# virtualsecureplatform/cuFHE

Measured on AMD Instinct MI355X. Metric: nand_gate_bootstraps_per_sec, higher is better.
Workload: dtype f64

## Files before the change

### cufhe_amd/csrc/kernels.hip.h

```cpp
#pragma once
#include "kernels_common.hip.h"

namespace cufhe_amd {

__global__ __launch_bounds__(kNttThreads) void bk_to_ntt_kernel(
    double* __restrict__ bk_ntt, const uint32_t* __restrict__ bk, size_t polys,
    const NttTables* __restrict__ gt, double n_inverse)
{
    extern __shared__ __attribute__((aligned(16))) char smem[];
    double* tabs = (double*)smem;
    load_tables_to_lds(tabs, gt);
    __syncthreads();
    const int wave = threadIdx.x >> 6, lane = threadIdx.x & 63;
    const size_t poly = (size_t)blockIdx.x * kNttWavesPerBlock + wave;
    if (poly >= polys) return;
    const WaveCtx ctx = make_wave_ctx(smem, kLdsTableBytes + wave * kTileBytes, 0, gt, lane);
    double x[kRegs];
#pragma unroll
    for (int r = 0; r < kRegs; r++) x[r] = (double)(int32_t)bk[poly * kN + lane + 64 * r];
    ntt_forward<false>(x, ctx);
    double2* dst = (double2*)(bk_ntt + poly * kN);
#pragma unroll
    for (int q = 0; q < 8; q++) {
        double2 v;
        v.x = fpf::reduce(fpf::mulmod_wide(x[2 * q], n_inverse));
        v.y = fpf::reduce(fpf::mulmod_wide(x[2 * q + 1], n_inverse));
        dst[q * 64 + lane] = v;
    }
}

__global__ __launch_bounds__(512) void clock_probe_kernel(double* __restrict__ hz_out, double* __restrict__ sink, int iters)
{
    double x = 1.0 + threadIdx.x * 1e-9, y = 0.5;
    const unsigned long long c0 = __builtin_amdgcn_s_memtime(), r0 = __builtin_amdgcn_s_memrealtime();
#pragma unroll 1
    for (int i = 0; i < iters; i++) {
#pragma unroll
        for (int k = 0; k < 16; k++) { x = __builtin_fma(x, 0.999999, y); y = __builtin_fma(y, 0.999999, x); }
    }
    const unsigned long long c1 = __builtin_amdgcn_s_memtime(), r1 = __builtin_amdgcn_s_memrealtime();
    if (x + y == 12345.678) sink[0] = x;
    if ((threadIdx.x & 63) == 0)
        hz_out[blockIdx.x * (blockDim.x >> 6) + (threadIdx.x >> 6)] = (double)(c1 - c0) / (double)(r1 - r0) * 1.0e8;
}

__device__ __forceinline__ void rotate_sub(uint32_t (&temp)[kRegs], const uint32_t (&acc)[kRegs],
                                           char* tile, int lane, uint32_t abar)
{
    const int alo = (int)(abar & (kN - 1));
    const bool ahi = (abar >> kNbit) != 0;
    char* wpos = tile + opaque(4 * lane + (ahi ? 0 : 4 * kN));
    char* wneg = tile + opaque(4 * lane + (ahi ? 4 * kN : 0));
    asm volatile("" ::: "memory");
#pragma unroll
    for (int r = 0; r < kRegs; r++) {
        *(uint32_t*)(wpos + 256 * r) = acc[r];
        *(uint32_t*)(wneg + 256 * r) = 0u - acc[r];
    }
    asm volatile("" ::: "memory");
    const char* rbase = tile + opaque(4 * (lane - alo + kN));
    uint32_t rot[kRegs];
#pragma unroll
    for (int r = 0; r < kRegs; r++) rot[r] = *(const uint32_t*)(rbase + 256 * r);
#pragma unroll
    for (int r = 0; r < kRegs; r++) temp[r] = (rot[r] - acc[r] + decomp_offset()) ^ decomp_signmask();
}

template <class SPEC, int R, bool LAST, bool FIRST = false>
__device__ __forceinline__ void product_into(double& acc, double x, double w)
{
    constexpr bool wide = r4::needs_wide(SPEC::in().v[R]);
    static_assert(!(LAST && FIRST), "a sum of one product has no first row apart from its last");
    if constexpr (LAST) acc = wide ? fpf::mulmod_add_wide(x, w, acc) : fpf::mulmod_add(x, w, acc);
    else if constexpr (FIRST) acc = wide ? fpf::mulmod_wide(x, w) : fpf::mulmod(x, w);
    else acc += wide ? fpf::mulmod_wide(x, w) : fpf::mulmod(x, w);
}
template <class SPEC, bool LAST, bool FIRST, int Q>
__device__ __forceinline__ void pointwise_piece(double (&A0)[kRegs], double (&A1)[kRegs], const double (&x)[kRegs], const double2& b)
{
    if constexpr (Q < 8) {
        product_into<SPEC, 2 * Q, LAST, FIRST>(A0[2 * Q], x[2 * Q], b.x);
        product_into<SPEC, 2 * Q + 1, LAST, FIRST>(A0[2 * Q + 1], x[2 * Q + 1], b.y);
    } else {
        product_into<SPEC, 2 * (Q - 8), LAST, FIRST>(A1[2 * (Q - 8)], x[2 * (Q - 8)], b.x);
        product_into<SPEC, 2 * (Q - 8) + 1, LAST, FIRST>(A1[2 * (Q - 8) + 1], x[2 * (Q - 8) + 1], b.y);
    }
}
template <class SPEC, bool LAST, bool FIRST, int Q = 0>
__device__ __forceinline__ void pointwise_pieces(double (&A0)[kRegs], double (&A1)[kRegs], const double (&x)[kRegs],
                                                 double2 (&b)[16], const char* row_lane)
{
#ifndef CUFHE_AMD_BK_DEPTH
#define CUFHE_AMD_BK_DEPTH 3
#endif
    constexpr int D = CUFHE_AMD_BK_DEPTH;
    if constexpr (Q < 16) {
        if constexpr (Q + D < 16) b[Q + D] = *(const double2*)(row_lane + (Q + D) * 1024);
        __builtin_amdgcn_sched_barrier(0x0006);
        pointwise_piece<SPEC, LAST, FIRST, Q>(A0, A1, x, b[Q]);
        __builtin_amdgcn_sched_barrier(0x0006);
        pointwise_pieces<SPEC, LAST, FIRST, Q + 1>(A0, A1, x, b, row_lane);
    }
}
template <class SPEC, bool LAST, bool FIRST = false>
__device__ __forceinline__ void pointwise_accumulate(double (&A0)[kRegs], double (&A1)[kRegs],
                                                     const double (&x)[kRegs], const char* row_lane)
{
#if defined(CUFHE_AMD_DIAGNOSTIC_BUILD) && defined(CUFHE_AMD_ABL_NO_BK)
    if constexpr (FIRST) {
#pragma unroll
        for (int r = 0; r < kRegs; r++) { A0[r] = 0.0; A1[r] = 0.0; }
    }
#pragma unroll
    for (int q = 0; q < 8; q++) {
        A0[2 * q] += fpf::mulmod_wide(x[2 * q], 1234567.0 + q);
        A0[2 * q + 1] += fpf::mulmod_wide(x[2 * q + 1], 7654321.0 + q);
        A1[2 * q] += fpf::mulmod_wide(x[2 * q], 2234567.0 + q);
        A1[2 * q + 1] += fpf::mulmod_wide(x[2 * q + 1], 8654321.0 + q);
    }
    (void)row_lane;
    return;
#endif
    constexpr int D = CUFHE_AMD_BK_DEPTH;
    double2 b[16];
#pragma unroll
    for (int q = 0; q < D; q++) b[q] = *(const double2*)(row_lane + q * 1024);
    pointwise_pieces<SPEC, LAST, FIRST>(A0, A1, x, b, row_lane);
}

#if defined(CUFHE_AMD_DIAGNOSTIC_BUILD) && defined(CUFHE_AMD_ABL_PHASES)
#define CUFHE_AMD_DIAG_ARG , unsigned long long& diag_wait
#define CUFHE_AMD_DIAG_PASS , diag_wait
#define CUFHE_AMD_ROW_SYNC(R) { const unsigned long long t0_ = __builtin_readcyclecounter(); pipe.sync(R); diag_wait += __builtin_readcyclecounter() - t0_; }
#else
#define CUFHE_AMD_DIAG_ARG
#define CUFHE_AMD_DIAG_PASS
#define CUFHE_AMD_ROW_SYNC(R) pipe.sync(R);
#endif
struct RowPipe {
    const char* src;
    char* buf;
    uint32_t voff;
    int wave, lane, total_rows;
    bool late;
    int row_off;
    __device__ __forceinline__ RowPipe(const char* bk, char* buf_, int wave_, int lane_, int total_rows_, bool late_)
        : src(bk + 2 * wave_ * 1024), buf(buf_), voff(lane_ * 16), wave(wave_), lane(lane_), total_rows(total_rows_), late(late_),
          row_off((kBkRowBuffers - 1) * kBkRowBytes) {}
    static __device__ __forceinline__ int next_off(int off) { return off == (kBkRowBuffers - 1) * kBkRowBytes ? 0 : off + kBkRowBytes; }
    __device__ __forceinline__ void issue(int R)
    {
        if (R < total_rows) {
            char* dst = buf + next_off(row_off) + 2 * wave * 1024;
#pragma unroll
            for (int c = 0; c < 2; c++) lds_dma16(src + c * 1024, voff, dst + c * 1024);
        }
        src += kBkRowBytes;
    }
    __device__ __forceinline__ void sync(int R)
    {
#if defined(CUFHE_AMD_DIAGNOSTIC_BUILD) && defined(CUFHE_AMD_ABL_NO_SYNC)
        (void)R;
        return;
#endif
        lds_dma_wait_all();
        __syncthreads();
        row_off = next_off(row_off);
        issue(R + 1);
    }
    __device__ __forceinline__ const char* row() const { return buf + opaque(row_off + lane * 16); }
};

using BrSpectrum = r4::FwdDigits<(1 << (kBgbit - 1))>::Spectrum;
using BrSums = r4::PointwiseSum<BrSpectrum, kBkRows, true>;
using BrInverse = r4::Inverse<BrSums>;
static_assert(r4::valid(BrSpectrum::in()) && r4::valid(BrSums::in()) && r4::valid(BrInverse::Out::in()),
              "blind_rotate_kernel: the lazy-reduction schedule of the CMux step exceeds the FP64 mantissa");

template <bool FIRST, bool LAST>
__device__ __forceinline__ void cmux_row(double (&A0)[kRegs], double (&A1)[kRegs], const uint32_t (&temp)[kRegs], int d,
                                         const WaveCtx& ctx, RowPipe& pipe, int row, const TuFwdPinned& tuf CUFHE_AMD_DIAG_ARG)
{
    constexpr int kDigitMax = 1 << (kBgbit - 1);
    const uint32_t pos = 32 - (d + 1) * kBgbit;
    double x[kRegs];
#pragma unroll
    for (int r = 0; r < kRegs; r++)
        x[r] = (double)(int32_t)__builtin_amdgcn_sbfe(temp[r], pos, (uint32_t)kBgbit);
    double twb[kTbCount];
    ntt_forward_digits_a_r4<kDigitMax, true>(x, ctx, &tuf, &twb);
    if (pipe.late) CUFHE_AMD_ROW_SYNC(row)
    ntt_forward_digits_bc_r4<kDigitMax, false, true>(x, ctx, twb);
    if (!pipe.late) CUFHE_AMD_ROW_SYNC(row)
    pointwise_accumulate<BrSpectrum, LAST, FIRST>(A0, A1, x, pipe.row());
}

template <bool FIRST_COMPONENT, bool LAST_COMPONENT>
__device__ __forceinline__ void cmux_component(double (&A0)[kRegs], double (&A1)[kRegs],
                                               const uint32_t (&accj)[kRegs], const WaveCtx& ctx,
                                               char* tile, int lane, uint32_t abar,
                                               RowPipe& pipe, int first_row, const TuFwdPinned& tuf CUFHE_AMD_DIAG_ARG)
{
    uint32_t temp[kRegs];
    rotate_sub(temp, accj, tile, lane, abar);
    static_assert(kL >= 2, "the first and the last row of a component are two rows");
    constexpr int lo = FIRST_COMPONENT ? 1 : 0, hi = LAST_COMPONENT ? kL - 1 : kL;
    if constexpr (FIRST_COMPONENT) cmux_row<true, false>(A0, A1, temp, 0, ctx, pipe, first_row, tuf CUFHE_AMD_DIAG_PASS);
#pragma unroll 1
    for (int d = lo; d < hi; d++) cmux_row<false, false>(A0, A1, temp, d, ctx, pipe, first_row + d, tuf CUFHE_AMD_DIAG_PASS);
    if constexpr (LAST_COMPONENT) cmux_row<false, true>(A0, A1, temp, kL - 1, ctx, pipe, first_row + kL - 1, tuf CUFHE_AMD_DIAG_PASS);
}

template <bool TWB_LOADED>
__device__ __forceinline__ void inverse_and_add(double (&A)[kRegs], uint32_t (&accj)[kRegs], const WaveCtx& ctx,
                                                const double (&twc)[kTcCount], double (&twb)[kTbCount])
{
    ntt_inverse_r4_tw<BrSums, false, TWB_LOADED>(A, ctx, twc, twb);
    lift_add<BrInverse::Out>(accj, A);
}

template <bool TABLE>
__global__ __launch_bounds__(kBrThreads, 2) void blind_rotate_kernel(
    const LinDesc* __restrict__ descs, int count, const double* __restrict__ bk_ntt,
    const NttTables* __restrict__ gt, int steps, uint32_t* __restrict__ acc_dump, int active, const uint32_t* __restrict__ tvs,
    const uint32_t* const* __restrict__ tables)
{
    extern __shared__ __attribute__((aligned(16))) char smem[];
    double* tabs = (double*)(smem + kBrLdsTables);
    load_packed_tables_to_lds(tabs, gt);
    const int wave = __builtin_amdgcn_readfirstlane(threadIdx.x >> 6);
    const int lane = threadIdx.x & 63;
    const int g = blockIdx.x * active + wave;
    char* tile = smem + kBrLdsTiles + wave * kTileBytes;
    uint16_t* abar_lds = (uint16_t*)(smem + kBrLdsAbar + wave * kAbarBytes);
    const WaveCtx ctx = make_wave_ctx_packed(smem, kBrLdsTiles + wave * kTileBytes, kBrLdsTables, gt, lane);
    RowPipe pipe((const char*)bk_ntt, smem + kBrLdsBk, wave, lane, steps * kBkRows, wave >= kBrWavesPerBlock / 2);
    pipe.issue(0);
    if (wave >= active || g >= count) {
        __syncthreads();
#pragma unroll 1
        for (int R = 0; R < pipe.total_rows; R++) pipe.sync(R);
        return;
    }

    const LinDesc d = descs[g];
    uint32_t bword = 0;
#pragma unroll
    for (int rr = 0; rr < 10; rr++) {
        const int i = lane + 64 * rr;
        uint32_t c = 0;
        if (i <= kLvl0N) c = (uint32_t)d.ca * d.in0[i] + (uint32_t)d.cb * d.in1[i];
        if (rr == 9) bword = c;
        if (i < kLvl0N) abar_lds[i] = (uint16_t)((c + (1u << (32 - 2 - kNbit))) >> (32 - 1 - kNbit));
    }
    bword = __builtin_amdgcn_readlane(bword, kLvl0N - 64 * 9) + d.off;
    const uint32_t bbar = 2 * kN - (bword >> (32 - 1 - kNbit));

    uint32_t acc0[kRegs], acc1[kRegs];
#pragma unroll
    for (int r = 0; r < kRegs; r++) {
        const uint32_t e = lane + 64 * r;
        acc0[r] = 0;
        const bool neg = (bbar != 2 * kN) && ((e < (bbar & (kN - 1))) != ((bbar >> kNbit) != 0));
        acc1[r] = neg ? 0u - kMu : kMu;
    }
    const uint32_t* tab = nullptr;
    if constexpr (TABLE) tab = tables[g];
    if (TABLE && tab) {
        const int s = desc_shift(d.pad);
        uint32_t bb = bbar;
        if (s) {
            for (int i = lane; i < kLvl0N; i += 64) abar_lds[i] = (uint16_t)ms_abar((uint32_t)d.ca * d.in0[i] + (uint32_t)d.cb * d.in1[i], s);
            bb = ms_bbar(bword, s);
        }
#pragma unroll
        for (int r = 0; r < kRegs; r++) {
            acc0[r] = rotated_tv_coef(tab, bb, lane + 64 * r);
            acc1[r] = rotated_tv_coef(tab + kN, bb, lane + 64 * r);
        }
    } else if (d.pad) {
        const uint32_t* tv = desc_tv(tvs, d.pad);
        const int s = desc_shift(d.pad);
        uint32_t bb = bbar;
        if (s) {
            for (int i = lane; i < kLvl0N; i += 64) abar_lds[i] = (uint16_t)ms_abar((uint32_t)d.ca * d.in0[i] + (uint32_t)d.cb * d.in1[i], s);
            bb = ms_bbar(bword, s);
        }
#pragma unroll
        for (int r = 0; r < kRegs; r++) acc1[r] = rotated_tv_coef(tv, bb, lane + 64 * r);
    }
    __syncthreads();
    TuFwdPinned tuf;
    tuf.load(gt);
#if defined(CUFHE_AMD_DIAGNOSTIC_BUILD) && defined(CUFHE_AMD_ABL_PHASES)
    unsigned long long diag_wait = 0;
    const unsigned long long diag_t0 = __builtin_readcyclecounter();
#endif

#pragma unroll 1
    for (int i = 0; i < steps; i++) {
        const uint32_t abar = __builtin_amdgcn_readfirstlane((uint32_t)abar_lds[i]);
        double A0[kRegs], A1[kRegs], inv_twc[kTcCount], inv_twb[kTbCount];
        cmux_component<true, false>(A0, A1, acc0, ctx, tile, lane, abar, pipe, i * kBkRows, tuf CUFHE_AMD_DIAG_PASS);
        cmux_component<false, true>(A0, A1, acc1, ctx, tile, lane, abar, pipe, i * kBkRows + kL, tuf CUFHE_AMD_DIAG_PASS);
        load_packed(inv_twc, ctx.tc_inv);
        inverse_and_add<false>(A0, acc0, ctx, inv_twc, inv_twb);
        inverse_and_add<true>(A1, acc1, ctx, inv_twc, inv_twb);
    }

    if (acc_dump) {
        uint32_t* o = acc_dump + (size_t)g * 2 * kN;
#pragma unroll
        for (int r = 0; r < kRegs; r++) {
            o[lane + 64 * r] = acc0[r];
            o[kN + lane + 64 * r] = acc1[r];
        }
#if defined(CUFHE_AMD_DIAGNOSTIC_BUILD) && defined(CUFHE_AMD_ABL_PHASES)
        if (lane == 0) {
            ((unsigned long long*)o)[0] = __builtin_readcyclecounter() - diag_t0;
            ((unsigned long long*)o)[1] = diag_wait;
        }
#endif
    }
    if (d.out) {
        uint32_t* o = d.out;
#pragma unroll
        for (int r = 0; r < kRegs; r++) {
            const int e = lane + 64 * r;
            if (e == 0) { o[0] = acc0[r]; o[kN] = acc1[r]; }
            else o[kN - e] = 0u - acc0[r];
        }
        if (const int s = desc_shift(d.pad)) {
#pragma unroll
            for (int r = 0; r < kRegs; r++) extract_more(o, 1 << s, lane + 64 * r, acc0[r], acc1[r]);
        }
    }
}

constexpr int kKsWaves = 16;
constexpr int kKsThreads = 64 * kKsWaves;
constexpr int kKsRowPad = 640;
constexpr int kKsPieces = 3;
constexpr int kKsStepBytes = kKsT * kKsNumBase * kKsRowPad * 4;
constexpr int kKsBuffers = 3;
constexpr int kKsDigitSteps = 1024;
constexpr int kKsLdsDigits = kKsWaves * kKsDigitSteps * 2;

struct KsShapeDefault {
    using Desc = LinDesc;
    static constexpr int kn = kN, t = kKsT, row_pad = kKsRowPad, n_out = kLvl0N;
    static constexpr uint32_t koff()
    {
        uint32_t o = 1u << (32 - (1 + kKsBasebit * kKsT));
        for (int i = 1; i <= kKsT; i++) o += ((1u << kKsBasebit) / 2) << (32 - i * kKsBasebit);
        return o;
    }
    static __device__ __forceinline__ uint32_t digit_word(const Desc& d, int j)
    {
        return ((uint32_t)d.ca * d.in0[j] + (uint32_t)d.cb * d.in1[j] + koff()) >> 16;
    }
    static __device__ __forceinline__ uint32_t bprime(const Desc& d) { return (uint32_t)d.ca * d.in0[kn] + (uint32_t)d.cb * d.in1[kn] + d.off; }
};
template <class S>
struct KsDims {
    static constexpr int pairs = (S::row_pad - 512) / 128;
    static constexpr int words = 8 + 2 * pairs;
    static constexpr int step_bytes = S::t * kKsNumBase * S::row_pad * 4;
    static constexpr int dma_pieces = step_bytes / 1024;
    static constexpr int dma_more = dma_pieces - 2 * kKsWaves;
    static constexpr int lds_bytes = kKsLdsDigits + kKsBuffers * step_bytes;
    static constexpr int min_slices = (S::kn + kKsDigitSteps - 1) / kKsDigitSteps;
    static_assert(S::row_pad == 512 || S::row_pad == 640, "a lane owns two quads and at most one pair of a row");
    static_assert(step_bytes % 1024 == 0 && dma_more >= 0 && dma_more <= kKsWaves, "two or three DMA pieces per wave and step");
    static_assert(S::t * kKsBasebit <= 16 && S::n_out < S::row_pad, "digit word of 16 bits; the output fits a row");
    static_assert(lds_bytes <= 160 * 1024, "digit words + three step buffers fit the CU's LDS");
};
static_assert(KsDims<KsShapeDefault>::step_bytes == kKsStepBytes && KsDims<KsShapeDefault>::lds_bytes == 155648, "BASELINE shape");

typedef uint32_t ks_u32x4 __attribute__((ext_vector_type(4)));
typedef uint32_t ks_u32x2 __attribute__((ext_vector_type(2)));
struct KsRow { ks_u32x4 a, b; ks_u32x2 c; };
template <int ROW1, int ROW2, int PAIRS>
__device__ __forceinline__ void ks_digit_load(const uint32_t f, const uint32_t a0, const uint32_t a1, const uint32_t a2, KsRow& r)
{
    if constexpr (PAIRS) {
        asm volatile(
            "s_cmp_eq_u32 %3, 2\n\t"
            "s_cbranch_scc1 .Lks_ld_end_%=\n\t"
            "s_cmp_eq_u32 %3, 0\n\t"
            "s_cbranch_scc1 .Lks_ld_two_%=\n\t"
            "ds_read_b128 %0, %4 offset:%7\n\t"
            "ds_read_b128 %1, %5 offset:%7\n\t"
            "ds_read_b64 %2, %6 offset:%7\n\t"
            "s_branch .Lks_ld_end_%=\n"
            ".Lks_ld_two_%=:\n\t"
            "ds_read_b128 %0, %4 offset:%8\n\t"
            "ds_read_b128 %1, %5 offset:%8\n\t"
            "ds_read_b64 %2, %6 offset:%8\n"
            ".Lks_ld_end_%=:"
            : "=&v"(r.a), "=&v"(r.b), "=&v"(r.c)
            : "s"(f), "v"(a0), "v"(a1), "v"(a2), "n"(ROW1), "n"(ROW2)
            : "memory", "scc");
    } else {
        asm volatile(
            "s_cmp_eq_u32 %2, 2\n\t"
            "s_cbranch_scc1 .Lks_ld_end_%=\n\t"
            "s_cmp_eq_u32 %2, 0\n\t"
            "s_cbranch_scc1 .Lks_ld_two_%=\n\t"
            "ds_read_b128 %0, %3 offset:%5\n\t"
            "ds_read_b128 %1, %4 offset:%5\n\t"
            "s_branch .Lks_ld_end_%=\n"
            ".Lks_ld_two_%=:\n\t"
            "ds_read_b128 %0, %3 offset:%6\n\t"
            "ds_read_b128 %1, %4 offset:%6\n"
            ".Lks_ld_end_%=:"
            : "=&v"(r.a), "=&v"(r.b)
            : "s"(f), "v"(a0), "v"(a1), "n"(ROW1), "n"(ROW2)
            : "memory", "scc");
    }
}
template <int PAIRS>
__device__ __forceinline__ void ks_digit_acc(const uint32_t f, const KsRow& r, uint32_t (&res)[8 + 2 * PAIRS])
{
    if constexpr (PAIRS) {
#define CUFHE_AMD_KS_ALL(OP)                                                                                               \
    OP " %0, %0, %11\n\t" OP " %1, %1, %12\n\t" OP " %2, %2, %13\n\t" OP " %3, %3, %14\n\t" OP " %4, %4, %15\n\t"             \
    OP " %5, %5, %16\n\t" OP " %6, %6, %17\n\t" OP " %7, %7, %18\n\t" OP " %8, %8, %19\n\t" OP " %9, %9, %20\n"
        asm volatile(
            "s_cmp_eq_u32 %10, 2\n\t"
            "s_cbranch_scc1 .Lks_acc_end_%=\n\t"
            "s_cmp_eq_u32 %10, 3\n\t"
            "s_cbranch_scc1 .Lks_acc_sub_%=\n\t"
            CUFHE_AMD_KS_ALL("v_add_u32_e32")
            "\ts_branch .Lks_acc_end_%=\n"
            ".Lks_acc_sub_%=:\n\t"
            CUFHE_AMD_KS_ALL("v_sub_u32_e32")
            ".Lks_acc_end_%=:"
            : "+v"(res[0]), "+v"(res[1]), "+v"(res[2]), "+v"(res[3]), "+v"(res[4]), "+v"(res[5]), "+v"(res[6]), "+v"(res[7]), "+v"(res[8]), "+v"(res[9])
            : "s"(f), "v"(r.a.x), "v"(r.a.y), "v"(r.a.z), "v"(r.a.w), "v"(r.b.x), "v"(r.b.y), "v"(r.b.z), "v"(r.b.w), "v"(r.c.x), "v"(r.c.y)
            : "scc");
#undef CUFHE_AMD_KS_ALL
    } else {
#define CUFHE_AMD_KS_ALL(OP)                                                                                               \
    OP " %0, %0, %9\n\t" OP " %1, %1, %10\n\t" OP " %2, %2, %11\n\t" OP " %3, %3, %12\n\t" OP " %4, %4, %13\n\t"              \
    OP " %5, %5, %14\n\t" OP " %6, %6, %15\n\t" OP " %7, %7, %16\n"
        asm volatile(
            "s_cmp_eq_u32 %8, 2\n\t"
            "s_cbranch_scc1 .Lks_acc_end_%=\n\t"
            "s_cmp_eq_u32 %8, 3\n\t"
            "s_cbranch_scc1 .Lks_acc_sub_%=\n\t"
            CUFHE_AMD_KS_ALL("v_add_u32_e32")
            "\ts_branch .Lks_acc_end_%=\n"
            ".Lks_acc_sub_%=:\n\t"
            CUFHE_AMD_KS_ALL("v_sub_u32_e32")
            ".Lks_acc_end_%=:"
            : "+v"(res[0]), "+v"(res[1]), "+v"(res[2]), "+v"(res[3]), "+v"(res[4]), "+v"(res[5]), "+v"(res[6]), "+v"(res[7])
            : "s"(f), "v"(r.a.x), "v"(r.a.y), "v"(r.a.z), "v"(r.a.w), "v"(r.b.x), "v"(r.b.y), "v"(r.b.z), "v"(r.b.w)
            : "scc");
#undef CUFHE_AMD_KS_ALL
    }
}
template <int I, int N, class F>
__device__ __forceinline__ void ks_for(F&& f)
{
    if constexpr (I < N) {
        f(std::integral_constant<int, I>{});
        ks_for<I + 1, N>(f);
    }
}
__device__ __forceinline__ uint32_t ks_field(const uint32_t dj, const int k) { return (dj >> (16 - (k + 1) * kKsBasebit)) & ((1u << kKsBasebit) - 1); }
template <class S>
__device__ __forceinline__ void ks_load_all(const uint32_t dj, const uint32_t (&pb)[3], KsRow (&r)[S::t])
{
// ... 401 lines not shown
```

### cufhe_amd/csrc/ntt_wave.h

```cpp
#pragma once
#include <hip/hip_runtime.h>
#include "fpfield.h"
#include "ntt_r4.h"
#include "ntt_tables.h"

namespace cufhe_amd {

constexpr int kRegs = 16;
constexpr int kTileSlots = 66 * 16;
constexpr int kTileBytes = kTileSlots * 8;

constexpr double forward_digit_spectrum_bound(double digit_max)
{
    const double s1 = digit_max * (1.0 + fpf::ROOT4 + fpf::ROOT8 + fpf::ROOT8 * fpf::ROOT8 * fpf::ROOT8);
    if (s1 >= 9007199254740992.0 / 64.0) return -1.0;
    double b = s1 / fpf::P;
    for (int s = 2; s <= 8; s++) {
        if (b >= fpf::LIM_NARROW) return -1.0;
        b = b + fpf::after_mulmod(b);
    }
    if (b >= fpf::LIM_WIDE) return -1.0;
    return b + fpf::after_mulmod_wide(b);
}
constexpr double forward_words_spectrum_bound()
{
    double b = 4294967296.0 / fpf::P;
    for (int s = 0; s <= 7; s++) {
        if (b >= fpf::LIM_NARROW) return -1.0;
        b = b + fpf::after_mulmod(b);
    }
    for (int s = 8; s <= 9; s++) {
        if (b >= fpf::LIM_WIDE) return -1.0;
        b = b + fpf::after_mulmod_wide(b);
    }
    return b;
}
static_assert(forward_words_spectrum_bound() > 0 && forward_words_spectrum_bound() < fpf::LIM_WIDE, "forward NTT schedule (32-bit words in)");
constexpr bool pointwise_sum_fits(double s, int rows)
{
    return s > 0 && s < fpf::LIM_WIDE && rows * fpf::after_mulmod_wide(s) < fpf::LIM_WIDE;
}
constexpr double inverse_output_bound()
{
    double b = 0.5001;
    for (int s = 0; s < 2; s++) {
        if (2 * b >= fpf::LIM_NARROW) return -1.0;
        b = 2 * b;
    }
    for (int half = 0; half < 2; half++) {
        if (2 * b >= fpf::LIM_NARROW) return -1.0;
        b = 2 * b;
        if (2 * b >= fpf::LIM_WIDE) return -1.0;
        b = 2 * b;
        b = 0.5001;
        for (int s = 0; s < 2; s++) {
            if (2 * b >= fpf::LIM_NARROW) return -1.0;
            b = 2 * b;
        }
    }
    return b;
}
constexpr bool inverse_schedule_fits() { return inverse_output_bound() > 0 && inverse_output_bound() < 2.57; }
static_assert(inverse_schedule_fits(), "inverse NTT lazy-reduction schedule exceeds the FP64 mantissa");


__device__ __forceinline__ void load_tables_to_lds(double* lds, const NttTables* g)
{
    const double* src = g->tb_fwd;
    for (int i = threadIdx.x; i < kLdsTableDoubles; i += blockDim.x) lds[i] = src[i];
}

__device__ __forceinline__ void load_packed_tables_to_lds(double* lds, const NttTables* g)
{
    const double* src = g->tbp_fwd;
    for (int i = threadIdx.x; i < kLdsTablePackedDoubles; i += blockDim.x) lds[i] = src[i];
}

struct WaveCtx {
    char* a65;
    char* a66;
    char* b65;
    char* b66;
    const char* tb_fwd;
    const char* tb_inv;
    const char* tc_fwd;
    const char* tc_inv;
    const NttTables* gt;
    const char* tu_l;
};

__device__ __forceinline__ void lds_dma16(const void* src, char* dst_uniform)
{
    const uint32_t base = (uint32_t)(uintptr_t)(__attribute__((address_space(3))) void*)dst_uniform;
#pragma clang diagnostic push
#pragma clang diagnostic ignored "-Winline-asm"
    asm volatile("s_mov_b32 m0, %1\n\ts_nop 0\n\tglobal_load_lds_dwordx4 %0, off" ::"v"(src), "s"(base) : "memory", "m0");
#pragma clang diagnostic pop
}
__device__ __forceinline__ void lds_dma16(const char* src_uniform, uint32_t voff, char* dst_uniform)
{
    const uint32_t base = (uint32_t)(uintptr_t)(__attribute__((address_space(3))) void*)dst_uniform;
#pragma clang diagnostic push
#pragma clang diagnostic ignored "-Winline-asm"
    asm volatile("s_mov_b32 m0, %2\n\ts_nop 0\n\tglobal_load_lds_dwordx4 %0, %1" ::"v"(voff), "s"(src_uniform), "s"(base) : "memory", "m0");
#pragma clang diagnostic pop
}
__device__ __forceinline__ void lds_dma_wait_all() { asm volatile("s_waitcnt vmcnt(0)" ::: "memory"); }

__device__ __forceinline__ int opaque(int off)
{
    asm volatile("" : "+v"(off));
    return off;
}

__device__ __forceinline__ WaveCtx make_wave_ctx(char* lds, int tile_off, int tables_off,
                                                 const NttTables* gt, int lane)
{
    const int lam = lane & 15, hi = lane >> 4;
    WaveCtx c;
    c.a65 = lds + opaque(tile_off + 8 * lane);
    c.a66 = c.a65;
    c.b65 = lds + opaque(tile_off + 8 * (65 * lam + hi));
    c.b66 = lds + opaque(tile_off + 8 * (66 * lam + hi));
    c.tb_fwd = lds + opaque(tables_off + 8 * lam);
    c.tb_inv = c.tb_fwd + 8 * (kTbCount * 16);
    c.tc_fwd = lds + opaque(tables_off + 8 * (2 * kTbCount * 16) + 8 * lane);
    c.tc_inv = c.tc_fwd + 8 * (kTcCount * 64);
    c.gt = gt;
    c.tu_l = nullptr;
    return c;
}

__device__ __forceinline__ WaveCtx make_wave_ctx_packed(char* lds, int tile_off, int tables_off, const NttTables* gt, int lane)
{
    WaveCtx c = make_wave_ctx(lds, tile_off, tables_off, gt, lane);
    c.tb_fwd = lds + opaque(tables_off + 8 * kTbpStride * (lane & 15));
    c.tb_inv = c.tb_fwd + 8 * 16 * kTbpStride;
    c.tc_fwd = lds + opaque(tables_off + 8 * 2 * 16 * kTbpStride + 8 * kTcpStride * lane);
    c.tc_inv = c.tc_fwd + 8 * 64 * kTcpStride;
    return c;
}
__device__ __forceinline__ double2 lds_ld2(const char* p, int off) { return *(const double2*)(p + off); }
template <int COUNT>
__device__ __forceinline__ void load_packed(double (&tw)[COUNT], const char* base)
{
#pragma unroll
    for (int i = 0; i < (COUNT + 1) / 2; i++) {
        const double2 v = lds_ld2(base, 16 * i);
        tw[2 * i] = v.x;
        if (2 * i + 1 < COUNT) tw[2 * i + 1] = v.y;
    }
}
#if defined(CUFHE_AMD_DIAGNOSTIC_BUILD) && defined(CUFHE_AMD_ABL_NO_TW)
__device__ __forceinline__ double lds_ld(const char* p, int off) { return 12345678.0 + (double)off + (double)(uintptr_t)p * 1e-30; }
#else
__device__ __forceinline__ double lds_ld(const char* p, int off) { return *(const double*)(p + off); }
#endif
__device__ __forceinline__ void lds_st(char* p, int off, double v) { *(double*)(p + off) = v; }

template <bool WIDE>
__device__ __forceinline__ void ct_bfly(double& a, double& b, double w)
{
    const double t = WIDE ? fpf::mulmod_wide(b, w) : fpf::mulmod(b, w);
    const double u = a;
    a = u + t;
    b = u - t;
}
template <bool WIDE>
__device__ __forceinline__ void gs_bfly(double& a, double& b, double w)
{
    const double u = a, v = b;
    a = u + v;
    b = WIDE ? fpf::mulmod_wide(u - v, w) : fpf::mulmod(u - v, w);
}

struct TwUniform {
    const double* t;
    __device__ __forceinline__ double operator()(int k) const { return t[k]; }
};
struct TwLane {
    const char* t;
    __device__ __forceinline__ double operator()(int k) const { return lds_ld(t, 128 * k); }
};

__device__ __forceinline__ void ct_bfly_exact(double& a, double& b, double w)
{
    const double u = a, v = b;
    a = __builtin_fma(v, w, u);
    b = __builtin_fma(-v, w, u);
}

__device__ __forceinline__ void ct_exact_first_two(double (&x)[kRegs], const double root4 = fpf::ROOT4, const double root8 = fpf::ROOT8)
{
    constexpr double kZ3 = fpf::ROOT8 * fpf::ROOT8 * fpf::ROOT8;
#pragma unroll
    for (int r = 0; r < 4; r++) {
        const double a = x[r], a1 = x[r + 4], b = x[r + 8], b1 = x[r + 12];
        const double u = __builtin_fma(b, root4, a), v = __builtin_fma(-b, root4, a);
        const double u1 = __builtin_fma(b1, root4, a1);
        const double t = __builtin_fma(a1, kZ3, b1 * fpf::ROOT8);
        x[r] = __builtin_fma(u1, root8, u);
        x[r + 4] = __builtin_fma(-u1, root8, u);
        x[r + 8] = v + t;
        x[r + 12] = v - t;
    }
}

template <bool SMALL_IN, class TW, bool EXACT0 = false>
__device__ __forceinline__ void ct_four_stages(double (&x)[kRegs], const TW& tw)
{
    if (SMALL_IN) {
        ct_exact_first_two(x);
    } else {
        const double w0 = tw(0);
#pragma unroll
        for (int r = 0; r < 8; r++) {
            if (EXACT0) ct_bfly_exact(x[r], x[r + 8], w0);
            else ct_bfly<false>(x[r], x[r + 8], w0);
        }
#pragma unroll
        for (int g = 0; g < 2; g++) {
            const double w = tw(1 + g);
#pragma unroll
            for (int r = 0; r < 4; r++) ct_bfly<false>(x[8 * g + r], x[8 * g + r + 4], w);
        }
    }
#pragma unroll
    for (int g = 0; g < 4; g++) {
        const double w = tw(3 + g);
#pragma unroll
        for (int r = 0; r < 2; r++) ct_bfly<false>(x[4 * g + r], x[4 * g + r + 2], w);
    }
#pragma unroll
    for (int g = 0; g < 8; g++) ct_bfly<false>(x[2 * g], x[2 * g + 1], tw(7 + g));
}
template <class TW>
__device__ __forceinline__ void gs_four_stages(double (&x)[kRegs], const TW& tw)
{
#pragma unroll
    for (int g = 0; g < 8; g++) gs_bfly<false>(x[2 * g], x[2 * g + 1], tw(7 + g));
#pragma unroll
    for (int g = 0; g < 4; g++) {
        const double w = tw(3 + g);
#pragma unroll
        for (int r = 0; r < 2; r++) gs_bfly<true>(x[4 * g + r], x[4 * g + r + 2], w);
    }
#pragma unroll
    for (int r = 0; r < 16; r++) x[r] = fpf::reduce(x[r]);
#pragma unroll
    for (int g = 0; g < 2; g++) {
        const double w = tw(1 + g);
#pragma unroll
        for (int r = 0; r < 4; r++) gs_bfly<false>(x[8 * g + r], x[8 * g + r + 4], w);
    }
    {
        const double w = tw(0);
#pragma unroll
        for (int r = 0; r < 8; r++) gs_bfly<false>(x[r], x[r + 8], w);
    }
}

template <int S, bool WIDE, class TW>
__device__ __forceinline__ void gs_stage(double (&x)[kRegs], const TW& tw, int first)
{
#pragma unroll
    for (int g = 0; g < 8 / S; g++) {
        const double w = tw(first + g);
#pragma unroll
        for (int r = 0; r < S; r++) gs_bfly<WIDE>(x[2 * S * g + r], x[2 * S * g + r + S], w);
    }
}
template <class TW>
__device__ __forceinline__ void gs_four_stages2(double (&x)[kRegs], double (&y)[kRegs], const TW& tw)
{
    gs_stage<1, false>(x, tw, 7);
    gs_stage<1, false>(y, tw, 7);
    gs_stage<2, true>(x, tw, 3);
    gs_stage<2, true>(y, tw, 3);
#pragma unroll
    for (int r = 0; r < 16; r++) x[r] = fpf::reduce(x[r]);
#pragma unroll
    for (int r = 0; r < 16; r++) y[r] = fpf::reduce(y[r]);
// ... 127 lines not shown
}
__device__ __forceinline__ void load_tu(double (&tu)[15], const char* tu_lds)
{
#pragma unroll
    for (int k = 0; k < 15; k++) tu[k] = lds_ld(tu_lds, 8 * k);
}
template <bool SMALL_IN, bool EXACT0 = false>
__device__ __forceinline__ void ntt_forward_a_tu(double (&x)[kRegs], const double (&tu)[15])
{
    ct_four_stages<SMALL_IN, TwArr, EXACT0>(x, TwArr{tu});
}
template <bool WIDE8, bool HALF_TILE = false>
__device__ __forceinline__ void ntt_forward_bc(double (&x)[kRegs], const WaveCtx& c)
{
    double twb[kTbCount];
#pragma unroll
    for (int k = 0; k < kTbCount; k++) twb[k] = lds_ld(c.tb_fwd, 128 * k);
    if (HALF_TILE) xpose_half_tile<true>(x, c.a66, c.b66);
    else CUFHE_AMD_XPOSE(c.a66, 8 * 66, c.b66, 32)
    ct_four_stages<false>(x, TwArr{twb});
    double twc[kTcCount];
#pragma unroll
    for (int k = 0; k < kTcCount; k++) twc[k] = lds_ld(c.tc_fwd, 512 * k);
    xpose_bc_permlane(x);
#pragma unroll
    for (int g = 0; g < 4; g++) {
#pragma unroll
        for (int r = 0; r < 2; r++) ct_bfly<WIDE8>(x[4 * g + r], x[4 * g + r + 2], twc[g]);
    }
#pragma unroll
    for (int g = 0; g < 8; g++) ct_bfly<true>(x[2 * g], x[2 * g + 1], twc[4 + g]);
}
template <bool SMALL_IN, bool HALF_TILE = false>
__device__ __forceinline__ void ntt_forward(double (&x)[kRegs], const WaveCtx& c)
{
    ntt_forward_a<SMALL_IN>(x, c);
    ntt_forward_bc<!SMALL_IN, HALF_TILE>(x, c);
}

template <bool HALF_TILE = false, bool TU_LDS = false>
__device__ __forceinline__ void ntt_inverse_twc(double (&x)[kRegs], const WaveCtx& c, const double (&twc)[kTcCount])
{
#pragma unroll
    for (int g = 0; g < 8; g++) gs_bfly<false>(x[2 * g], x[2 * g + 1], twc[4 + g]);
#pragma unroll
    for (int g = 0; g < 4; g++) {
#pragma unroll
        for (int r = 0; r < 2; r++) gs_bfly<false>(x[4 * g + r], x[4 * g + r + 2], twc[g]);
    }
    double twb[kTbCount];
#pragma unroll
    for (int k = 0; k < kTbCount; k++) twb[k] = lds_ld(c.tb_inv, 128 * k);
    xpose_cb_permlane(x);
    gs_four_stages(x, TwArr{twb});
    double tu[15];
    if (TU_LDS) load_tu(tu, c.tu_l + 128);
    if (HALF_TILE) xpose_half_tile<false>(x, c.a65, c.b65);
    else CUFHE_AMD_XPOSE(c.b65, 32, c.a65, 8 * 65)
    if (TU_LDS) gs_four_stages(x, TwArr{tu});
    else gs_four_stages(x, TwUniform{c.gt->tu_inv});
}
template <bool HALF_TILE = false, bool TU_LDS = false>
__device__ __forceinline__ void ntt_inverse2_twc(double (&x)[kRegs], double (&y)[kRegs], const WaveCtx& c, const double (&twc)[kTcCount])
{
    gs_stage<1, false>(x, TwArr{twc}, 4);
    gs_stage<1, false>(y, TwArr{twc}, 4);
    gs_stage<2, false>(x, TwArr{twc}, 0);
    gs_stage<2, false>(y, TwArr{twc}, 0);
    double twb[kTbCount];
#pragma unroll
    for (int k = 0; k < kTbCount; k++) twb[k] = lds_ld(c.tb_inv, 128 * k);
    xpose_cb_permlane(x);
    xpose_cb_permlane(y);
    gs_four_stages2(x, y, TwArr{twb});
    double tu[15];
    if (TU_LDS) load_tu(tu, c.tu_l + 128);
    if (HALF_TILE) { xpose_half_tile<false>(x, c.a65, c.b65); xpose_half_tile<false>(y, c.a65, c.b65); }
    else { CUFHE_AMD_XPOSE(c.b65, 32, c.a65, 8 * 65) { double (&x)[kRegs] = y; CUFHE_AMD_XPOSE(c.b65, 32, c.a65, 8 * 65) } }
    if (TU_LDS) gs_four_stages2(x, y, TwArr{tu});
    else gs_four_stages2(x, y, TwUniform{c.gt->tu_inv});
}
template <bool HALF_TILE = false, bool TU_LDS = false>
__device__ __forceinline__ void ntt_inverse(double (&x)[kRegs], const WaveCtx& c)
{
    double twc[kTcCount];
#pragma unroll
    for (int k = 0; k < kTcCount; k++) twc[k] = lds_ld(c.tc_inv, 512 * k);
    ntt_inverse_twc<HALF_TILE, TU_LDS>(x, c, twc);
}



struct TuFwdPinned {
    double t[12];
    double root4, root8;
    __device__ __forceinline__ void load(const NttTables* gt)
    {
#pragma unroll
        for (int k = 0; k < 12; k++) {
            double v = gt->tu_fwd[3 + k];
            asm volatile("" : "+s"(v));
            t[k] = v;
        }
        root4 = fpf::ROOT4;
        root8 = fpf::ROOT8;
        asm volatile("" : "+s"(root4), "+s"(root8));
    }
    __device__ __forceinline__ double operator()(int k) const { return t[k - 3]; }
};
template <int DIGIT_MAX, bool STORE = false, class TW = TwUniform>
__device__ __forceinline__ void ntt_forward_digits_a_r4(double (&x)[kRegs], const WaveCtx& c, const TW* pinned = nullptr, double (*twb_ahead)[kTbCount] = nullptr)
{
    using A0 = typename r4::FwdDigits<DIGIT_MAX>::A0;
    if constexpr (!STORE) {
        ct_exact_first_two(x);
        r4::ct_pass_lo<A0, 3, 7>(x, TwUniform{c.gt->tu_fwd});
    } else {
        const TW& tw = *pinned;
        ct_exact_first_two(x, tw.root4, tw.root8);
        if (twb_ahead) load_packed(*twb_ahead, c.tb_fwd);
        asm volatile("" ::: "memory");
        r4::Group<A0, false, 0>::ct(x, tw(3), tw(7), tw(8));
#pragma unroll
        for (int r = 0; r < 4; r++) lds_st(c.a66, 8 * 66 * r, x[r]);
        r4::Group<A0, false, 1>::ct(x, tw(4), tw(9), tw(10));
#pragma unroll
        for (int r = 4; r < 8; r++) lds_st(c.a66, 8 * 66 * r, x[r]);
        r4::Group<A0, false, 2>::ct(x, tw(5), tw(11), tw(12));
#pragma unroll
        for (int r = 8; r < 12; r++) lds_st(c.a66, 8 * 66 * r, x[r]);
        r4::Group<A0, false, 3>::ct(x, tw(6), tw(13), tw(14));
#pragma unroll
        for (int r = 12; r < 16; r++) lds_st(c.a66, 8 * 66 * r, x[r]);
    }
}
template <int DIGIT_MAX, bool HALF_TILE = false, bool STORED = false>
__device__ __forceinline__ void ntt_forward_digits_bc_r4(double (&x)[kRegs], const WaveCtx& c, const double* twb_loaded = nullptr)
{
    using F = r4::FwdDigits<DIGIT_MAX>;
    static_assert(r4::valid(F::Spectrum::in()), "radix-4 forward transform of gadget digits: a value exceeds 2^53");
    static_assert(!(HALF_TILE && STORED), "the half-size tile takes the layout change in two passes");
    double twb[kTbCount];
    if (twb_loaded) {
#pragma unroll
        for (int k = 0; k < kTbCount; k++) twb[k] = twb_loaded[k];
    } else {
        load_packed(twb, c.tb_fwd);
    }
    if (HALF_TILE) xpose_half_tile<true>(x, c.a66, c.b66);
    else if (STORED) {
        asm volatile("" ::: "memory");
#pragma unroll
        for (int r = 0; r < kRegs; r++) x[r] = lds_ld(c.b66, 32 * r);
    }
    else CUFHE_AMD_XPOSE(c.a66, 8 * 66, c.b66, 32)
    r4::ct_pass_hi<typename F::B0>(x, TwArr{twb});
    r4::ct_pass_lo<typename F::B1, 3, 7>(x, TwArr{twb});
    double twc[kTcCount];
    load_packed(twc, c.tc_fwd);
    xpose_bc_permlane(x);
    r4::reduce_mask<F::kReduceC>(x);
    r4::ct_pass_lo<typename F::C1, 0, 4>(x, TwArr{twc});
}

template <class S0, bool HALF_TILE, bool TWB_LOADED>
__device__ __forceinline__ void ntt_inverse_r4_tw(double (&x)[kRegs], const WaveCtx& c, const double (&twc)[kTcCount], double (&twb)[kTbCount]);
template <class S0, bool HALF_TILE = false>
__device__ __forceinline__ void ntt_inverse_r4(double (&x)[kRegs], const WaveCtx& c)
{
    double twc[kTcCount], twb[kTbCount];
    load_packed(twc, c.tc_inv);
    ntt_inverse_r4_tw<S0, HALF_TILE, false>(x, c, twc, twb);
}
template <class S0, bool HALF_TILE, bool TWB_LOADED>
__device__ __forceinline__ void ntt_inverse_r4_tw(double (&x)[kRegs], const WaveCtx& c, const double (&twc)[kTcCount], double (&twb)[kTbCount])
{
    using V = r4::Inverse<S0>;
    static_assert(r4::valid(V::Out::in()), "radix-4 inverse transform: a value exceeds 2^53");
    r4::gs_pass_lo<S0, 0, 4>(x, TwArr{twc});
    r4::reduce_above<typename V::C1, V::kLimit>(x);
    if (!TWB_LOADED) load_packed(twb, c.tb_inv);
    xpose_cb_permlane(x);
    r4::gs_pass_lo<typename V::B0, 3, 7>(x, TwArr{twb});
    r4::reduce_above<r4::AfterGs<typename V::B0, false>, V::kLimit>(x);
    if (HALF_TILE) {
        r4::gs_pass_hi<typename V::B1>(x, TwArr{twb});
        r4::reduce_above<r4::AfterGs<typename V::B1, true>, V::kLimit>(x);
        xpose_half_tile<false>(x, c.a65, c.b65);
    } else {
        using B1o = r4::AfterGs<typename V::B1, true>;
        const double w = twb[0], v = twb[1], vw = twb[2];
        double tu[15];
#pragma unroll
        for (int k = 0; k < 15; k++) tu[k] = c.gt->tu_inv[k];
        asm volatile("" ::: "memory");
        r4::Group<typename V::B1, true, 0>::gs(x, w, v, vw);
        r4::reduce_above_group<B1o, V::kLimit, 0>(x);
#pragma unroll
        for (int k = 0; k < 16; k += 4) lds_st(c.b65, 32 * k, x[k]);
        r4::Group<typename V::B1, true, 1>::gs(x, w, v, vw);
        r4::reduce_above_group<B1o, V::kLimit, 1>(x);
#pragma unroll
        for (int k = 1; k < 16; k += 4) lds_st(c.b65, 32 * k, x[k]);
        r4::Group<typename V::B1, true, 2>::gs(x, w, v, vw);
        r4::reduce_above_group<B1o, V::kLimit, 2>(x);
#pragma unroll
        for (int k = 2; k < 16; k += 4) lds_st(c.b65, 32 * k, x[k]);
        r4::Group<typename V::B1, true, 3>::gs(x, w, v, vw);
        r4::reduce_above_group<B1o, V::kLimit, 3>(x);
#pragma unroll
        for (int k = 3; k < 16; k += 4) lds_st(c.b65, 32 * k, x[k]);
        asm volatile("" ::: "memory");
#pragma unroll
        for (int r = 0; r < kRegs; r++) x[r] = lds_ld(c.a65, 8 * 65 * r);
        r4::gs_pass_lo<typename V::A0, 3, 7>(x, TwArr{tu});
        r4::reduce_above<r4::AfterGs<typename V::A0, false>, V::kLimit>(x);
        r4::gs_pass_hi<typename V::A1>(x, TwArr{tu});
        return;
    }
    r4::gs_pass_lo<typename V::A0, 3, 7>(x, TwUniform{c.gt->tu_inv});
    r4::reduce_above<r4::AfterGs<typename V::A0, false>, V::kLimit>(x);
    r4::gs_pass_hi<typename V::A1>(x, TwUniform{c.gt->tu_inv});
}
template <class OUT, int R = 0>
__device__ __forceinline__ void lift_add(uint32_t (&acc)[kRegs], const double (&x)[kRegs])
{
    if constexpr (R < kRegs) {
        if constexpr (OUT::in().v[R] < 2.57) acc[R] += fpf::lift_u32_small(x[R]);
        else acc[R] += fpf::lift_u32(x[R]);
        lift_add<OUT, R + 1>(acc, x);
    }
}

}
```

Before: 114,800.

## Interleave the two inverse NTTs so LDS transpose reads overlap butterfly work

The two per-step inverse transforms with lift-add (one per accumulator component) were run back to back. They are now one fused routine that splits each inverse NTT into front, LDS-read request and back stages, then interleaves them. The LDS transpose reads of one polynomial are meant to be in flight while the other polynomial's butterflies execute, hiding LDS latency. The uniform twiddles are pinned in scalar registers. This raises register pressure, and it depends on in-order LDS ordering because both polynomials share the same tile. Diagnostic-only LDS wait counters are also added, but they compile out by default.

```diff
diff --git a/cufhe_amd/csrc/kernels.hip.h b/cufhe_amd/csrc/kernels.hip.h
--- a/cufhe_amd/csrc/kernels.hip.h
+++ b/cufhe_amd/csrc/kernels.hip.h
@@ -45,7 +45,7 @@
 }
 
 __device__ __forceinline__ void rotate_sub(uint32_t (&temp)[kRegs], const uint32_t (&acc)[kRegs],
-                                           char* tile, int lane, uint32_t abar)
+                                           char* tile, int lane, uint32_t abar CUFHE_AMD_DIAG_LDS_ARG)
 {
     const int alo = (int)(abar & (kN - 1));
     const bool ahi = (abar >> kNbit) != 0;
@@ -62,6 +62,8 @@
     uint32_t rot[kRegs];
 #pragma unroll
     for (int r = 0; r < kRegs; r++) rot[r] = *(const uint32_t*)(rbase + 256 * r);
+    CUFHE_AMD_DIAG_LDS_WAIT(diag, kDiagWaitRotate)
+    CUFHE_AMD_DIAG_LDS_WAIT(diag, kDiagWaitEmpty)
 #pragma unroll
     for (int r = 0; r < kRegs; r++) temp[r] = (rot[r] - acc[r] + decomp_offset()) ^ decomp_signmask();
 }
@@ -104,7 +106,7 @@
 }
 template <class SPEC, bool LAST, bool FIRST = false>
 __device__ __forceinline__ void pointwise_accumulate(double (&A0)[kRegs], double (&A1)[kRegs],
-                                                     const double (&x)[kRegs], const char* row_lane)
+                                                     const double (&x)[kRegs], const char* row_lane CUFHE_AMD_DIAG_LDS_ARG)
 {
 #if defined(CUFHE_AMD_DIAGNOSTIC_BUILD) && defined(CUFHE_AMD_ABL_NO_BK)
     if constexpr (FIRST) {
@@ -125,6 +127,7 @@
     double2 b[16];
 #pragma unroll
     for (int q = 0; q < D; q++) b[q] = *(const double2*)(row_lane + q * 1024);
+    CUFHE_AMD_DIAG_LDS_WAIT(diag, kDiagWaitRow)
     pointwise_pieces<SPEC, LAST, FIRST>(A0, A1, x, b, row_lane);
 }
 
@@ -192,7 +195,7 @@
     if (pipe.late) CUFHE_AMD_ROW_SYNC(row)
     ntt_forward_digits_bc_r4<kDigitMax, false, true>(x, ctx, twb);
     if (!pipe.late) CUFHE_AMD_ROW_SYNC(row)
-    pointwise_accumulate<BrSpectrum, LAST, FIRST>(A0, A1, x, pipe.row());
+    pointwise_accumulate<BrSpectrum, LAST, FIRST>(A0, A1, x, pipe.row() CUFHE_AMD_DIAG_LDS_PASS(ctx));
 }
 
 template <bool FIRST_COMPONENT, bool LAST_COMPONENT>
@@ -202,7 +205,7 @@
                                                RowPipe& pipe, int first_row, const TuFwdPinned& tuf CUFHE_AMD_DIAG_ARG)
 {
     uint32_t temp[kRegs];
-    rotate_sub(temp, accj, tile, lane, abar);
+    rotate_sub(temp, accj, tile, lane, abar CUFHE_AMD_DIAG_LDS_PASS(ctx));
     static_assert(kL >= 2, "the first and the last row of a component are two rows");
     constexpr int lo = FIRST_COMPONENT ? 1 : 0, hi = LAST_COMPONENT ? kL - 1 : kL;
     if constexpr (FIRST_COMPONENT) cmux_row<true, false>(A0, A1, temp, 0, ctx, pipe, first_row, tuf CUFHE_AMD_DIAG_PASS);
@@ -233,7 +236,13 @@
     const int g = blockIdx.x * active + wave;
     char* tile = smem + kBrLdsTiles + wave * kTileBytes;
     uint16_t* abar_lds = (uint16_t*)(smem + kBrLdsAbar + wave * kAbarBytes);
+#if defined(CUFHE_AMD_DIAGNOSTIC_BUILD) && defined(CUFHE_AMD_ABL_PHASES)
+    unsigned long long diag_lds[kDiagWaitKinds] = {};
+    WaveCtx ctx = make_wave_ctx_packed(smem, kBrLdsTiles + wave * kTileBytes, kBrLdsTables, gt, lane);
+    ctx.diag = diag_lds;
+#else
     const WaveCtx ctx = make_wave_ctx_packed(smem, kBrLdsTiles + wave * kTileBytes, kBrLdsTables, gt, lane);
+#endif
     RowPipe pipe((const char*)bk_ntt, smem + kBrLdsBk, wave, lane, steps * kBkRows, wave >= kBrWavesPerBlock / 2);
     pipe.issue(0);
     if (wave >= active || g >= count) {
@@ -300,12 +309,11 @@
 #pragma unroll 1
     for (int i = 0; i < steps; i++) {
         const uint32_t abar = __builtin_amdgcn_readfirstlane((uint32_t)abar_lds[i]);
-        double A0[kRegs], A1[kRegs], inv_twc[kTcCount], inv_twb[kTbCount];
+        double A0[kRegs], A1[kRegs], inv_twc[kTcCount];
         cmux_component<true, false>(A0, A1, acc0, ctx, tile, lane, abar, pipe, i * kBkRows, tuf CUFHE_AMD_DIAG_PASS);
         cmux_component<false, true>(A0, A1, acc1, ctx, tile, lane, abar, pipe, i * kBkRows + kL, tuf CUFHE_AMD_DIAG_PASS);
         load_packed(inv_twc, ctx.tc_inv);
-        inverse_and_add<false>(A0, acc0, ctx, inv_twc, inv_twb);
-        inverse_and_add<true>(A1, acc1, ctx, inv_twc, inv_twb);
+        ntt_inverse2_r4_lift<BrSums>(A0, A1, acc0, acc1, ctx, inv_twc);
     }
 
     if (acc_dump) {
@@ -319,6 +327,7 @@
         if (lane == 0) {
             ((unsigned long long*)o)[0] = __builtin_readcyclecounter() - diag_t0;
             ((unsigned long long*)o)[1] = diag_wait;
+            for (int k = 0; k < kDiagWaitKinds; k++) ((unsigned long long*)o)[2 + k] = diag_lds[k];
         }
 #endif
     }
diff --git a/cufhe_amd/csrc/ntt_wave.h b/cufhe_amd/csrc/ntt_wave.h
--- a/cufhe_amd/csrc/ntt_wave.h
+++ b/cufhe_amd/csrc/ntt_wave.h
@@ -87,7 +87,27 @@
     const char* tc_inv;
     const NttTables* gt;
     const char* tu_l;
+#if defined(CUFHE_AMD_DIAGNOSTIC_BUILD) && defined(CUFHE_AMD_ABL_PHASES)
+    unsigned long long* diag;
+#endif
 };
+#if defined(CUFHE_AMD_DIAGNOSTIC_BUILD) && defined(CUFHE_AMD_ABL_PHASES)
+enum { kDiagWaitFwdAB = 0, kDiagWaitRow, kDiagWaitRotate, kDiagWaitInvBA, kDiagWaitEmpty, kDiagWaitKinds };
+#define CUFHE_AMD_DIAG_LDS_WAIT(DIAG, KIND)                                                     \
+    if (DIAG) {                                                                                 \
+        __builtin_amdgcn_sched_barrier(0);       \
+        const unsigned long long t0_ = __builtin_readcyclecounter();                            \
+        asm volatile("s_waitcnt lgkmcnt(0)" ::: "memory");                                      \
+        (DIAG)[KIND] += __builtin_readcyclecounter() - t0_;                                     \
+        __builtin_amdgcn_sched_barrier(0);                                                      \
+    }
+#define CUFHE_AMD_DIAG_LDS_ARG , unsigned long long* diag = nullptr
+#define CUFHE_AMD_DIAG_LDS_PASS(C) , (C).diag
+#else
+#define CUFHE_AMD_DIAG_LDS_WAIT(DIAG, KIND)
+#define CUFHE_AMD_DIAG_LDS_ARG
+#define CUFHE_AMD_DIAG_LDS_PASS(C)
+#endif
 
 __device__ __forceinline__ void lds_dma16(const void* src, char* dst_uniform)
 {
@@ -128,6 +148,9 @@
     c.tc_inv = c.tc_fwd + 8 * (kTcCount * 64);
     c.gt = gt;
     c.tu_l = nullptr;
+#if defined(CUFHE_AMD_DIAGNOSTIC_BUILD) && defined(CUFHE_AMD_ABL_PHASES)
+    c.diag = nullptr;
+#endif
     return c;
 }
 
@@ -561,6 +584,7 @@
         asm volatile("" ::: "memory");
 #pragma unroll
         for (int r = 0; r < kRegs; r++) x[r] = lds_ld(c.b66, 32 * r);
+        CUFHE_AMD_DIAG_LDS_WAIT(c.diag, kDiagWaitFwdAB)
     }
     else CUFHE_AMD_XPOSE(c.a66, 8 * 66, c.b66, 32)
     r4::ct_pass_hi<typename F::B0>(x, TwArr{twb});
@@ -622,6 +646,7 @@
         asm volatile("" ::: "memory");
 #pragma unroll
         for (int r = 0; r < kRegs; r++) x[r] = lds_ld(c.a65, 8 * 65 * r);
+        CUFHE_AMD_DIAG_LDS_WAIT(c.diag, kDiagWaitInvBA)
         r4::gs_pass_lo<typename V::A0, 3, 7>(x, TwArr{tu});
         r4::reduce_above<r4::AfterGs<typename V::A0, false>, V::kLimit>(x);
         r4::gs_pass_hi<typename V::A1>(x, TwArr{tu});
@@ -641,4 +666,78 @@
     }
 }
 
-}
+template <class S0>
+__device__ __forceinline__ void ntt_inverse_r4_front(double (&x)[kRegs], const WaveCtx& c, const double (&twb)[kTbCount])
+{
+    using V = r4::Inverse<S0>;
+    using B1o = r4::AfterGs<typename V::B1, true>;
+    r4::gs_pass_lo<typename V::B0, 3, 7>(x, TwArr{twb});
+    r4::reduce_above<r4::AfterGs<typename V::B0, false>, V::kLimit>(x);
+    const double w = twb[0], v = twb[1], vw = twb[2];
+    asm volatile("" ::: "memory");
+    r4::Group<typename V::B1, true, 0>::gs(x, w, v, vw);
+    r4::reduce_above_group<B1o, V::kLimit, 0>(x);
+#pragma unroll
+    for (int k = 0; k < 16; k += 4) lds_st(c.b65, 32 * k, x[k]);
+    r4::Group<typename V::B1, true, 1>::gs(x, w, v, vw);
+    r4::reduce_above_group<B1o, V::kLimit, 1>(x);
+#pragma unroll
+    for (int k = 1; k < 16; k += 4) lds_st(c.b65, 32 * k, x[k]);
+    r4::Group<typename V::B1, true, 2>::gs(x, w, v, vw);
+    r4::reduce_above_group<B1o, V::kLimit, 2>(x);
+#pragma unroll
+    for (int k = 2; k < 16; k += 4) lds_st(c.b65, 32 * k, x[k]);
+    r4::Group<typename V::B1, true, 3>::gs(x, w, v, vw);
+    r4::reduce_above_group<B1o, V::kLimit, 3>(x);
+#pragma unroll
+    for (int k = 3; k < 16; k += 4) lds_st(c.b65, 32 * k, x[k]);
+    asm volatile("" ::: "memory");
+}
+__device__ __forceinline__ void ntt_inverse_r4_request(double (&x)[kRegs], const WaveCtx& c)
+{
+#pragma unroll
+    for (int r = 0; r < kRegs; r++) x[r] = lds_ld(c.a65, 8 * 65 * r);
+    asm volatile("" ::: "memory");
+    __builtin_amdgcn_sched_barrier(0);
+}
+template <class S0>
+__device__ __forceinline__ void ntt_inverse_r4_back(double (&x)[kRegs], const double (&tu)[15])
+{
+    using V = r4::Inverse<S0>;
+    r4::gs_pass_lo<typename V::A0, 3, 7>(x, TwArr{tu});
+    r4::reduce_above<r4::AfterGs<typename V::A0, false>, V::kLimit>(x);
+    r4::gs_pass_hi<typename V::A1>(x, TwArr{tu});
+}
+template <class S0>
+__device__ __forceinline__ void ntt_inverse2_r4_lift(double (&x)[kRegs], double (&y)[kRegs], uint32_t (&accx)[kRegs], uint32_t (&accy)[kRegs],
+                                                     const WaveCtx& c, const double (&twc)[kTcCount])
+{
+    using V = r4::Inverse<S0>;
+    static_assert(r4::valid(V::Out::in()), "radix-4 inverse transform: a value exceeds 2^53");
+    double tu[15], twb[kTbCount];
+#pragma unroll
+    for (int k = 0; k < 15; k++) tu[k] = c.gt->tu_inv[k];
+    load_packed(twb, c.tb_inv);
+    __builtin_amdgcn_sched_barrier(0);
+    r4::gs_pass_lo<S0, 0, 4>(x, TwArr{twc});
+    r4::reduce_above<typename V::C1, V::kLimit>(x);
+#pragma unroll
+    for (int k = 0; k < 15; k++) asm volatile("" : "+s"(tu[k]));
+    xpose_cb_permlane(x);
+    ntt_inverse_r4_front<S0>(x, c, twb);
+    ntt_inverse_r4_request(x, c);
+    r4::gs_pass_lo<S0, 0, 4>(y, TwArr{twc});
+    r4::reduce_above<typename V::C1, V::kLimit>(y);
+    xpose_cb_permlane(y);
+    ntt_inverse_r4_front<S0>(y, c, twb);
+    CUFHE_AMD_DIAG_LDS_WAIT(c.diag, kDiagWaitInvBA)
+    ntt_inverse_r4_request(y, c);
+    ntt_inverse_r4_back<S0>(x, tu);
+    lift_add<typename V::Out>(accx, x);
+    __builtin_amdgcn_sched_barrier(0);
+    CUFHE_AMD_DIAG_LDS_WAIT(c.diag, kDiagWaitInvBA)
+    ntt_inverse_r4_back<S0>(y, tu);
+    lift_add<typename V::Out>(accy, y);
+}
+
+}
```

New measurement: 115,400, median of 6. No clear change (+0.5%).
